# Orca0917/TransformerTTS

Measured on AMD Instinct MI355X. Metric: mel frames/sec teacher-forced step, LJSpeech-shape batch, 1/2/4/8 MI355X, higher is better.
Workload: dtype f32

## Files before the change

### include/ttts_hip.h

```cpp
#ifndef TTTS_HIP_H
#define TTTS_HIP_H

#include <stddef.h>
#include <stdint.h>

#ifdef __cplusplus
extern "C" {
#endif

#define TTTS_OK 0
#define TTTS_ERR_INVALID (-1)
#define TTTS_ERR_LAUNCH (-2)

#define TTTS_AMAX_SLOTS 1024

#define TTTS_ACT_NONE 0
#define TTTS_ACT_RELU 1
#define TTTS_ACT_TANH 2

typedef struct ttts_step_state {
    uint64_t seed;
    float lr;
    float p_tf;
    int64_t step;
// ... 225 lines not shown
                       size_t ws_bytes, int64_t* durations, uint8_t* valid, void* stream);
int ttts_heads_pad_w(const float* src, int64_t ld_src, float* dst, int64_t rows, int H, int head_dim, int width, void* stream);
int ttts_heads_unpad_w(const float* src, float* dst, int64_t ld_dst, int64_t rows, int H, int head_dim, int width, void* stream);
int ttts_attention_fwd_img(const void* q, const void* k, const void* v, const float* q_inv, const float* k_inv,
                           const float* v_inv, float* o, float* lse, float* attn, const int64_t* key_lens, int B, int H, int Tq,
                           int Tk, int ldq, int ldk, int ldv, int ldo, int causal, float q_scale, float drop_p, uint64_t seed,
                           const uint64_t* step_seed, const float* v_amax, float* o_amax_out, float* rowstat_out, int64_t q_inv_rows, int64_t k_inv_rows, int64_t stat_plane,
                           void* stream);
int ttts_attention_bwd_img(const void* q, const void* k, const void* v, const float* q_inv, const float* k_inv,
                           const float* v_inv, const float* o, const float* d_o, const float* rowstat, float* delta, float* dq,
                           float* dk, float* dv, const int64_t* key_lens, int B, int H, int Tq, int Tk, int ldq, int ldk, int ldv,
                           int ldo, int lddq, int lddk, int lddv, int causal, float q_scale, float drop_p, uint64_t seed,
                           const uint64_t* step_seed, const float* do_amax, float* dq_amax_out, float* dkv_amax_out,
                           float* dkv_partials , int q_splits ,
                           int64_t q_inv_rows, int64_t k_inv_rows, int64_t stat_plane, void* stream);

int ttts_embedding_fwd(const int64_t* ids, const float* table, float* out, int64_t n, int vocab, int d,
                       float* out_amax_out , void* stream);
int ttts_embedding_bwd(const int64_t* ids, const float* dout, float* dtable, int64_t n, int vocab, int d, int accumulate,
                       void* stream);
int ttts_posenc_fwd(const float* x, const float* pe, const float* alpha, float* y, int B, int T, int d, float drop_p,
                    uint64_t seed, const uint64_t* step_seed, float* y_amax_out , void* stream);
size_t ttts_posenc_bwd_workspace_bytes(void);
int ttts_posenc_bwd(const float* dy, const float* pe, float* dx, float* dalpha, float* ws, size_t ws_bytes, int B, int T,
                    int d, float drop_p, uint64_t seed, const uint64_t* step_seed, int accumulate, void* stream);
int ttts_relu_dropout_bwd(const float* dy, const float* out, float* dx, int64_t n, float drop_p, float* dx_amax_out,
                          void* stream);
int ttts_dropout_bwd(const float* dy, float* dx, int64_t n, float drop_p, uint64_t seed, const uint64_t* step_seed,
                     float* dx_amax_out, void* stream);
int ttts_zero(void* p, size_t nbytes, void* stream);
// ... 71 lines not shown
```

### transformertts_amd/_lib.py

```python
from __future__ import annotations

import ctypes
import os
from ctypes import c_char_p, c_float, c_int, c_int64, c_size_t, c_uint64, c_void_p

import torch

_HERE = os.path.dirname(os.path.abspath(__file__))
LIB_PATH = os.environ.get("TTTS_LIB", os.path.join(_HERE, "libttts_hip.so"))

P, I, L, F, U, Z = c_void_p, c_int, c_int64, c_float, c_uint64, c_size_t

SIGNATURES = {
    "ttts_last_error": (c_char_p, []),
    "ttts_abi_version": (I, []),
    "ttts_linear_fwd": (I, [P, P, P, P, P, L, I, I, I, F, U, P, I, I, P]),
    "ttts_linear_bwd_data": (I, [P, P, P, P, L, I, I, P, F, P]),
    "ttts_wgrad_workspace_bytes": (Z, [L, I, I, I]),
    "ttts_linear_bwd_weight": (I, [P, P, P, P, P, Z, L, I, I, I, I, I, P, P]),
    "ttts_split_bytes": (Z, [L, L]),
    "ttts_split_image_bytes": (Z, [L, L, I, I, I]),
    "ttts_gemm_tile_choice": (I, [L, I, I, I]),
    "ttts_weight_split": (I, [P, P, I, I, I, I, I, P]),
    "ttts_weight_split_units": (L, [L, L, I, I]),
# ... 37 lines not shown
    "ttts_bn_apply_fwd": (I, [P, P, P, P, P, P, L, I, I, F, U, P, P, P]),
    "ttts_bn_bwd": (I, [P, P, P, P, P, P, P, P, P, P, Z, L, I, I, F, U, P, I, P, I, P]),
    "ttts_layernorm_fwd": (I, [P, P, P, P, P, P, L, I, F, P, P, P, P]),
    "ttts_layernorm_bwd_workspace_bytes": (Z, [I]),
    "ttts_layernorm_bwd": (I, [P, P, P, P, P, P, P, P, P, Z, L, I, I, P, P, P, P]),
    "ttts_layernorm_bwd_drop": (I, [P, P, P, P, P, P, P, P, P, Z, L, I, I, P, F, U, P, P, P, P, P, P]),
    "ttts_attention_fwd": (I, [P, P, P, P, P, P, P, I, I, I, I, I, I, I, I, I, F, F, U, P, P]),
    "ttts_attention_fwd_x6": (I, [P, P, P, P, P, P, P, I, I, I, I, I, I, I, I, I, F, F, U, P, P]),
    "ttts_attention_fwd_h3": (I, [P, P, P, P, P, P, P, I, I, I, I, I, I, I, I, I, F, F, U, P, P, P, P, P, P, P]),
    "ttts_attention_bwd": (I, [P, P, P, P, P, P, P, P, P, P, P, I, I, I, I, I, I, I, I, I, I, I, I, F, F, U, P, P]),
    "ttts_attention_bwd_x6": (I, [P, P, P, P, P, P, P, P, P, P, P, I, I, I, I, I, I, I, I, I, I, I, I, F, F, U, P, P]),
    "ttts_attention_bwd_h3": (I, [P, P, P, P, P, P, P, P, P, P, P, I, I, I, I, I, I, I, I, I, I, I, I, F, F, U, P, P, P, P, P, P, P, P, P]),
    "ttts_attention_fwd_img": (I, [P, P, P, P, P, P, P, P, P, P, I, I, I, I, I, I, I, I, I, F, F, U, P, P, P, P, L, L, L, P]),
    "ttts_attention_bwd_img": (I, [P, P, P, P, P, P, P, P, P, P, P, P, P, P, I, I, I, I, I, I, I, I, I, I, I, I, F, F, U, P, P, P, P,
                                   P, I, L, L, L, P]),
    "ttts_attention_fwd_wide": (I, [P, P, P, P, P, P, P, I, I, I, I, I, I, I, I, I, F, F, U, P, P]),
    "ttts_attention_bwd_wide": (I, [P, P, P, P, P, P, P, P, P, P, P, I, I, I, I, I, I, I, I, I, I, I, I, F, F, U, P, P]),
    "ttts_attention_fwd_wide_masked": (I, [P, P, P, P, P, P, P, I, I, I, I, I, I, I, I, I, F, F, U, P, P, L, L, L, P, L, P]),
    "ttts_attention_bwd_wide_masked": (I, [P, P, P, P, P, P, P, P, P, P, P, I, I, I, I, I, I, I, I, I, I, I, I, F, F, U, P, P, L, L, L,
                                           P, L, P]),
    "ttts_attention_bwd_wide_dattn": (I, [P, P, P, P, P, P, P, P, P, P, P, I, I, I, I, I, I, I, I, I, I, I, I, F, F, U, P, P, L, L, L,
                                          P, L, P, P, L, L, L, P]),
    "ttts_guided_attention_fwd": (I, [P, P, P, U, F, I, I, I, I, P, I, I, I, P, P]),
    "ttts_guided_attention_bwd": (I, [P, P, P, U, F, I, I, I, I, I, I, P, P]),
    "ttts_alignment_rowstats": (I, [P, L, L, L, P, P, I, I, I, I, I, I, P, P, P, P]),
    "ttts_alignment_select": (I, [P, P, P, I, I, I, I, I, I, P, P, P]),
    "ttts_alignment_durations_argmax": (I, [P, P, P, P, I, I, I, I, I, P, P, P]),
    "ttts_alignment_mas_workspace_bytes": (Z, [I, I, I]),
    "ttts_alignment_mas": (I, [P, I, L, L, L, P, P, P, I, I, I, I, P, Z, P, P, P]),
    "ttts_heads_pad": (I, [P, L, P, L, I, I, P]),
# ... 76 lines not shown
```

### transformertts_amd/csrc/attention_common.h

```cpp
#pragma once
#include "ttts_common.h"

namespace ttts {

constexpr int HD = 64;
constexpr int KT_LD = HD + 1;
constexpr int WHD = 128;
constexpr int WLD = WHD + 1;
constexpr int QB = 128;
constexpr float NEG_INF = -__builtin_inff();
__device__ __forceinline__ float fast_exp2(float x) { return __builtin_amdgcn_exp2f(x); }
typedef unsigned int u32x4v __attribute__((ext_vector_type(4)));

struct RowSrc {
    __amdgpu_buffer_rsrc_t rsrc;
    int ld;
};
__device__ __forceinline__ RowSrc row_src(const float* base, long nrows, int ld) {
    RowSrc r;
    r.rsrc = __builtin_amdgcn_make_buffer_rsrc(const_cast<float*>(base), 0, (uint32_t)(nrows * ld * 4), 0x00020000);
    r.ld = ld;
    return r;
}
__device__ __forceinline__ float4 row_load4(const RowSrc& s, long row, int c4) {
// ... 209 lines not shown
    float m = 0.f;
#pragma unroll
    for (int r = 0; r < 16; ++r) m = fmaxf(m, fabsf(ds[r]));
    m = fmaxf(m, __shfl_xor(m, 32, 64));
    const uint32_t e = (__float_as_uint(m) >> 23) & 0xffu;
    const bool change = e >= 24u && e < 255u && (sds == 0.f || m * sds > 8192.f);
    if (__any(change)) {
        const float snew = change ? __uint_as_float((265u - e) << 23) : sds;
        const float f = (change && sds != 0.f) ? snew / sds : 1.f;
#pragma unroll
        for (int r = 0; r < 16; ++r) { acc[0][r] *= f; acc[1][r] *= f; }
        sds = snew;
    }
}

__device__ __forceinline__ void load_lane_frags_h3(const float* scratch, int l31, int half, float scale, f16x8v (&f)[4][2]) {
#pragma unroll
    for (int st = 0; st < 4; ++st) {
        float x[8];
#pragma unroll
        for (int e = 0; e < 8; ++e) x[e] = scratch[l31 * KT_LD + 16 * st + 8 * half + e];
        split_frag8_h3(x, scale, f[st][0], f[st][1]);
    }
}

static inline int attn_check(const char* name, int width, int B, int H, int Tq, int Tk, int ldq, int ldk, int ldv, int ldo,
                             int causal, float drop_p) {
    TTTS_REQUIRE(B > 0 && H > 0 && Tq > 0 && Tk > 0, "%s: sizes must be positive (B %d, H %d, Tq %d, Tk %d)", name, B, H, Tq, Tk);
    TTTS_REQUIRE((long)B * H < (1L << 31) && cdiv(Tq, QB) <= 65535 && cdiv(Tk, QB) <= 65535,
                 "%s: grid too large (B*H %ld, Tq %d, Tk %d)", name, (long)B * H, Tq, Tk);
// ... 59 lines not shown
```

### transformertts_amd/csrc/attention_img.hip

```cpp
#include "attention_common.h"

namespace ttts {

struct AttnImgArgs {
    const void* q; const void* k; const void* v;
    const float* q_inv; const float* k_inv; const float* v_inv;
    long q_rows, k_rows;
    long stat_plane;
    float* o; float* lse; float* attn;
    const float* dout; float* delta; float* dq; float* dk; float* dv;
    const int64_t* key_lens;
    int B, H, Tq, Tk;
    int ldq, ldk, ldv, ldo, lddq, lddk, lddv;
    float qscale;
    float drop_scale; uint32_t thr; uint64_t seed; const uint64_t* step_seed;
    const float* v_amax;
    const float* do_amax;
    float* amax_dq; float* amax_dkv;
    float* dkv_part; long part_stride;
    int ldp;
    float* o_amax;
    float* rowstat;
};

__device__ __forceinline__ uint32_t lds_addr_a(const void* p) {
    return (uint32_t)(uintptr_t)(__attribute__((address_space(3))) const void*)p;
}
typedef unsigned int u32x4a __attribute__((ext_vector_type(4)));
__device__ __forceinline__ void dma16a(u32x4a rsrc, uint32_t voff, uint32_t soff, uint32_t lds_dst) {
    uint32_t keep;
    asm volatile("s_mov_b32 %0, m0\n\ts_mov_b32 m0, %3\n\ts_nop 0\n\tbuffer_load_dwordx4 %1, %2, %4 offen lds\n\ts_mov_b32 m0, %0"
                 : "=&s"(keep) : "v"(voff), "s"(rsrc), "s"(lds_dst), "s"(soff) : "memory");
}
__device__ __forceinline__ void dma4a(u32x4a rsrc, uint32_t voff, uint32_t lds_dst) {
    uint32_t keep;
    asm volatile("s_mov_b32 %0, m0\n\ts_mov_b32 m0, %3\n\ts_nop 0\n\tbuffer_load_dword %1, %2, 0 offen lds\n\ts_mov_b32 m0, %0"
                 : "=&s"(keep) : "v"(voff), "s"(rsrc), "s"(lds_dst) : "memory");
}
__device__ __forceinline__ u32x4a make_rsrc(const void* base, uint32_t bytes) {
    const uint64_t a = reinterpret_cast<uint64_t>(base);
    return u32x4a{(uint32_t)a, (uint32_t)(a >> 32) & 0xffffu, bytes, 0x00020000u};
}

constexpr int IMG_PLANE = 64 * 128;
constexpr int IMG_TILE = 2 * IMG_PLANE;
__device__ __forceinline__ int isw(int r) { return ((r & 2) << 1) | ((r >> 2) & 3); }
typedef short s16x4v __attribute__((ext_vector_type(4)));
__device__ __forceinline__ s16x4v lds_tr4(const char* p) {
    return __builtin_amdgcn_ds_read_tr16_b64_v4i16(
        (__attribute__((address_space(3))) s16x4v*)(uintptr_t)lds_addr_a(p));
}
// ... 792 lines not shown
        const float fin = (sds > 0.f) ? a.qscale / sds : 0.f;
        float mx = 0.f;
#pragma unroll
        for (int r = 0; r < 16; ++r) {
            dq[0][r] *= fin; dq[1][r] *= fin;
            mx = fmaxf(mx, fmaxf(fabsf(dq[0][r]), fabsf(dq[1][r])));
        }
        if (a.amax_dq != nullptr) amax_publish(qg < a.Tq ? mx : 0.f, a.amax_dq, blockIdx.y * gridDim.x + blockIdx.x);
    }
    wave_store_rows4(dq, scratch4, a.dq + (long)b * a.Tq * a.lddq + h * HD, qw0, a.Tq, a.lddq, lane);
}

constexpr int DKI_QS = 32;
constexpr int DKI_PLANE = DKI_QS * 128;
constexpr int DKI_STAGE = 4 * DKI_PLANE + 5 * 256;
template <bool CAUSAL>
__global__ __launch_bounds__(256, 2) void attn_bwd_dkv_img_kernel(AttnImgArgs a) {
    const uint64_t seed_eff = site_seed(a.seed, a.step_seed);
    const uint32_t thr16 = a.thr << 16;
    __shared__ __attribute__((aligned(16))) char xs[(2 * DKI_STAGE > OUT_BYTES) ? 2 * DKI_STAGE : OUT_BYTES];
    __shared__ float red4[4];

    const int tid = threadIdx.x, lane = tid & 63;
    const int wave = __builtin_amdgcn_readfirstlane(tid >> 6);
    const int l31 = lane & 31, half = lane >> 5;
    const int kblk = blockIdx.y;
    const int h = blockIdx.x % a.H, b = blockIdx.x / a.H;
    const int k0 = kblk * QB, kw0 = k0 + wave * 32;
    const int kg = kw0 + l31;
    const uint32_t key_mult = attn_drop_mult((uint32_t)kg);
    float* scratch4 = reinterpret_cast<float*>(xs) + wave * 32 * OUT_LD;
// ... 14 lines not shown
#pragma unroll
            for (int p = 0; p < 2; ++p) {
                kf[s][p] = *reinterpret_cast<const f16x8v*>(kp + p * 128 + (2 * s + half) * 16);
                vf[s][p] = *reinterpret_cast<const f16x8v*>(vp + p * 128 + (2 * s + half) * 16);
            }
    }
    const float kinv = a.k_inv[(long)h * a.k_rows + (long)b * a.Tk + krow];
    const float vinv = a.v_inv[(long)h * a.k_rows + (long)b * a.Tk + krow];

    f32x16 dk[2], dv[2];
#pragma unroll
    for (int r = 0; r < 16; ++r) { dk[0][r] = 0.f; dk[1][r] = 0.f; dv[0][r] = 0.f; dv[1][r] = 0.f; }

    const float dp_unscale = inv_g * vinv * a.drop_scale;
    float sds = 0.f;
    const int nqs_all = (a.Tq + DKI_QS - 1) / DKI_QS;
    const int per_z = (nqs_all + (int)gridDim.z - 1) / (int)gridDim.z;
    const int nqs = min(nqs_all, ((int)blockIdx.z + 1) * per_z);
    int qs_begin = max(attn_qs_begin<CAUSAL, DKI_QS>(k0, klen, nqs), (int)blockIdx.z * per_z);
    if (qs_begin > nqs) qs_begin = nqs;

    const u32x4a rsQ = make_rsrc(reinterpret_cast<const char*>(a.q) + ((long)AIMG_SB(b) * a.Tq * a.ldq + AIMG_SH(h) * HD) * 4, (uint32_t)a.Tq * (uint32_t)a.ldq * 4u);
    const u32x4a rsG = make_rsrc(a.dout + (long)AIMG_SB(b) * a.Tq * a.ldo + AIMG_SH(h) * HD, (uint32_t)a.Tq * (uint32_t)a.ldo * 4u);
    const long plane = a.stat_plane;
    const u32x4a rsS0 = make_rsrc(a.rowstat + arow, (uint32_t)a.Tq * 4u), rsS1 = make_rsrc(a.rowstat + plane + arow, (uint32_t)a.Tq * 4u);
    const u32x4a rsS3 = make_rsrc(a.rowstat + 3 * plane + arow, (uint32_t)a.Tq * 4u), rsS4 = make_rsrc(a.rowstat + 4 * plane + arow, (uint32_t)a.Tq * 4u);
    const u32x4a rsD = make_rsrc(a.delta + arow, (uint32_t)a.Tq * 4u);
    const uint32_t lds0 = lds_addr_a(xs);
    const int ld_r = lane >> 3;
    const uint32_t ld_cq = (uint32_t)((lane & 7) ^ isw(8 * (wave & 1) + ld_r)) * 16u;
// ... 127 lines not shown
                const float4 f4 = *reinterpret_cast<const float4*>(stat + 256 + 2 * r + 4 * half);
                const float dl4[4] = {d4.x, d4.y, d4.z, d4.w}, cq4[4] = {f4.x, f4.y, f4.z, f4.w};
#pragma unroll
                for (int e = 0; e < 4; ++e) {
                    float g = dp[r + e] * dp_unscale;
                    float pk = pd[r + e];
                    {
                        const bool keep = attn_keep_word(hq[e], key_mult, thr16);
                        g = keep ? g : 0.f;
                        pk = keep ? pk : 0.f;
                    }
                    ds[r + e] = pd[r + e] * (g - dl4[e]) * cq4[e];
                    pd[r + e] = pk;
                }
            }
            attn_h3_track_scale(ds, sds, dk);
#pragma unroll
            for (int t2 = 0; t2 < 2; ++t2) {
                float x[8];
                f16x8v f[2];
#pragma unroll
                for (int e = 0; e < 8; ++e) x[e] = pd[8 * t2 + e];
                split_frag8_h3(x, H3A_P, f[0], f[1]);
#pragma unroll
                for (int i2 = 0; i2 < 2; ++i2) {
                    f16x8v af[2];
#pragma unroll
                    for (int pl = 0; pl < 2; ++pl) {
                        const char* gb = st_ + (2 + pl) * DKI_PLANE + t2 * 2048;
                        af[pl] = join_tr(lds_tr4(gb + t_off[i2][0]), lds_tr4(gb + t_off[i2][1]));
// ... 42 lines not shown

__global__ __launch_bounds__(256) void attn_dkv_reduce_kernel(const float* __restrict__ part, float* __restrict__ out, long n4, int zs,
                                                              long stride, float* __restrict__ amax, int cols4, long out_ld) {
    float mx = 0.f;
    for (long i = (long)blockIdx.x * blockDim.x + threadIdx.x; i < n4; i += (long)gridDim.x * blockDim.x) {
        float4 acc = reinterpret_cast<const float4*>(part)[i];
        for (int z = 1; z < zs; ++z) {
            const float4 v = reinterpret_cast<const float4*>(part + (long)z * stride)[i];
            acc.x += v.x; acc.y += v.y; acc.z += v.z; acc.w += v.w;
        }
        const long row = i / cols4;
        *reinterpret_cast<float4*>(out + row * out_ld + (i - row * cols4) * 4) = acc;
        mx = fmaxf(fmaxf(mx, fmaxf(fabsf(acc.x), fabsf(acc.y))), fmaxf(fabsf(acc.z), fabsf(acc.w)));
    }
    if (amax != nullptr) amax_publish(mx, amax, blockIdx.x * 4 + (threadIdx.x >> 6));
}

#ifndef TTTS_AIMG_KT
#define TTTS_AIMG_KT 32
#endif

static int check_img_spans(const char* name, int Tq, int Tk, int ldq, int ldk, int ldv) {
    TTTS_REQUIRE((uint64_t)Tq * ldq * 4 < (1ull << 32) && (uint64_t)Tk * ldk * 4 < (1ull << 32) && (uint64_t)Tk * ldv * 4 < (1ull << 32),
                 "%s: one utterance's operand exceeds 4 GiB", name);
    return TTTS_OK;
}
static int fill_img_planes(const char* name, AttnImgArgs& a, int B, int H, int Tq, int Tk, int64_t q_inv_rows, int64_t k_inv_rows,
                           int64_t stat_plane) {
    TTTS_REQUIRE((q_inv_rows == 0 || q_inv_rows >= (int64_t)B * Tq) && (k_inv_rows == 0 || k_inv_rows >= (int64_t)B * Tk) &&
                 (stat_plane == 0 || stat_plane >= (int64_t)B * H * Tq), "%s: plane strides smaller than the batch", name);
// ... 32 lines not shown
    a.o = o; a.lse = lse; a.attn = attn;
    a.v_amax = v_amax; a.o_amax = o_amax_out; a.rowstat = rowstat_out;
    dim3 grid(B * H, cdiv(Tq, QB), 1);
    if (causal)
        hipLaunchKernelGGL((attn_fwd_img_kernel<true, false, TTTS_AIMG_KT>), grid, dim3(256), 0, (hipStream_t)stream, a);
    else if (!attn)
        hipLaunchKernelGGL((attn_fwd_img_kernel<false, false, TTTS_AIMG_KT>), grid, dim3(256), 0, (hipStream_t)stream, a);
    else if (Tk <= 128)
        hipLaunchKernelGGL(attn_fwd_img_maps_kernel, grid, dim3(256), 0, (hipStream_t)stream, a);
    else
        hipLaunchKernelGGL((attn_fwd_img_kernel<false, true, 64>), grid, dim3(256), 0, (hipStream_t)stream, a);
    TTTS_LAUNCH_CHECK("attn_fwd_img_kernel");
    return TTTS_OK;
}

extern "C" int ttts_attention_bwd_img(const void* q, const void* k, const void* v, const float* q_inv, const float* k_inv,
                                      const float* v_inv, const float* o, const float* d_o, const float* rowstat, float* delta,
                                      float* dq, float* dk, float* dv, const int64_t* key_lens, int B, int H, int Tq, int Tk, int ldq,
                                      int ldk, int ldv, int ldo, int lddq, int lddk, int lddv, int causal, float q_scale,
                                      float drop_p, uint64_t seed, const uint64_t* step_seed, const float* do_amax,
                                      float* dq_amax_out, float* dkv_amax_out, float* dkv_partials, int q_splits,
                                      int64_t q_inv_rows, int64_t k_inv_rows, int64_t stat_plane, void* stream_) {
    hipStream_t stream = (hipStream_t)stream_;
    TTTS_REQUIRE(q && k && v && q_inv && k_inv && v_inv && o && d_o && rowstat && delta && dq && dk && dv && key_lens && do_amax,
                 "attention_bwd_img: null pointer");
    int rc = attn_check("attention_bwd_img", HD, B, H, Tq, Tk, ldq, ldk, ldv, ldo, causal, drop_p);
    if (!rc) rc = check_img_spans("attention_bwd_img", Tq, Tk, ldq, ldk, ldv);
    if (!rc) rc = attn_check_grad_strides("attention_bwd_img", HD, H, lddq, lddk, lddv);
    if (rc) return rc;
    TTTS_REQUIRE((((uintptr_t)q | (uintptr_t)k | (uintptr_t)v | (uintptr_t)o | (uintptr_t)d_o | (uintptr_t)do_amax) & 15) == 0,
                 "attention_bwd_img: q/k/v/o/d_o/do_amax must be 16-byte aligned");
    TTTS_REQUIRE((uint64_t)Tq * ldo * 4 < (1ull << 32), "attention_bwd_img: one utterance's d_o exceeds 4 GiB");
    AttnImgArgs a = {};
    attn_fill(a, key_lens, B, H, Tq, Tk, ldq, ldk, ldv, ldo, q_scale, drop_p, seed, step_seed);
    rc = fill_img_planes("attention_bwd_img", a, B, H, Tq, Tk, q_inv_rows, k_inv_rows, stat_plane);
    if (rc) return rc;
    a.q = q; a.k = k; a.v = v; a.q_inv = q_inv; a.k_inv = k_inv; a.v_inv = v_inv;
    a.o = const_cast<float*>(o); a.dout = d_o; a.delta = delta; a.dq = dq; a.dk = dk; a.dv = dv;
    a.lddq = lddq; a.lddk = lddk; a.lddv = lddv;
    a.do_amax = do_amax; a.amax_dq = dq_amax_out; a.amax_dkv = dkv_amax_out;
    a.rowstat = const_cast<float*>(rowstat);
    TTTS_REQUIRE(q_splits >= 1 && q_splits <= 16, "attention_bwd_img: q_splits out of 1..16");
    if (q_splits > 1) {
        TTTS_REQUIRE(dkv_partials && dv == dk + H * HD && lddk >= 2 * H * HD && lddv == lddk,
                     "attention_bwd_img: query splits need a workspace and a (dk | dv) gradient whose rows hold dk then dv");
        a.ldp = 2 * H * HD;
        a.dkv_part = dkv_partials; a.part_stride = (long)B * Tk * a.ldp;
    }
    rc = ATTN_LAUNCH_BWD(attn_bwd_dq_img_kernel, 0, attn_bwd_dkv_img_kernel, 0, causal, "attention_bwd_img", "attn_bwd_dq_img_kernel",
                         "attn_bwd_dkv_img_kernel", a, q_splits, stream);
    if (rc) return rc;
    if (q_splits > 1) {
        const long n4 = a.part_stride / 4;
        const long blocks = (n4 + 255) / 256;
        hipLaunchKernelGGL(attn_dkv_reduce_kernel, dim3((unsigned)(blocks < 2048 ? blocks : 2048)), dim3(256), 0, stream, dkv_partials, dk, n4,
                           q_splits, a.part_stride, dkv_amax_out, a.ldp / 4, (long)lddk);
        TTTS_LAUNCH_CHECK("attn_dkv_reduce_kernel");
    }
    return TTTS_OK;
}
```

### transformertts_amd/csrc/elementwise.hip

```cpp
#include <stdarg.h>

#include "ttts_common.h"

namespace ttts {

static thread_local char g_err[512] = "";
void set_error(const char* fmt, ...) {
    va_list ap;
    va_start(ap, fmt);
    vsnprintf(g_err, sizeof(g_err), fmt, ap);
    va_end(ap);
}

static inline int ew_grid(long n_items) {
    long g = (n_items + 255) / 256;
    if (g > 2048) g = 2048;
    if (g < 1) g = 1;
    return (int)g;
}

__global__ __launch_bounds__(256) void zero_kernel(uint32_t* __restrict__ p, long n) {
    const long head = (long)(((16 - (reinterpret_cast<uintptr_t>(p) & 15)) & 15) >> 2) < n ? (long)(((16 - (reinterpret_cast<uintptr_t>(p) & 15)) & 15) >> 2) : n;
    const long n4 = (n - head) / 4;
    uint4* q = reinterpret_cast<uint4*>(p + head);
// ... 311 lines not shown
    if (lane == 0) red[wave][1024] = accb;
    __syncthreads();
    for (int c = threadIdx.x; c < d; c += 256)
        ws[(long)blockIdx.x * (d + 1) + c] = (red[0][c] + red[1][c]) + (red[2][c] + red[3][c]);
    if (threadIdx.x == 0)
        ws[(long)blockIdx.x * (d + 1) + d] = (red[0][1024] + red[1][1024]) + (red[2][1024] + red[3][1024]);
}

}

using namespace ttts;

extern "C" {

const char* ttts_last_error(void) { return ttts::g_err; }
int ttts_abi_version(void) { return 21; }

int ttts_zero(void* p, size_t nbytes, void* stream) { return ::ttts::launch_zero(p, nbytes, (hipStream_t)stream); }

int ttts_heads_pad(const float* src, int64_t ld_src, float* dst, int64_t rows, int H, int head_dim, void* stream) {
    TTTS_REQUIRE(src && dst && rows > 0 && H > 0 && head_dim > 0 && head_dim <= 64 && ld_src >= (int64_t)H * head_dim,
                 "heads_pad: bad arguments (head_dim %d must be in 1..64)", head_dim);
    hipLaunchKernelGGL(heads_pad_kernel<64>, dim3(ew_grid(rows * H * 64)), dim3(256), 0, (hipStream_t)stream, src, (long)ld_src, dst,
                       (long)rows, H, head_dim, 0, 0L);
    TTTS_LAUNCH_CHECK("heads_pad_kernel");
    return TTTS_OK;
}

int ttts_heads_unpad(const float* src, float* dst, int64_t ld_dst, int64_t rows, int H, int head_dim, void* stream) {
    TTTS_REQUIRE(src && dst && rows > 0 && H > 0 && head_dim > 0 && head_dim <= 64 && ld_dst >= (int64_t)H * head_dim,
                 "heads_unpad: bad arguments (head_dim %d must be in 1..64)", head_dim);
// ... 144 lines not shown
```

### transformertts_amd/ops.py

```python
from __future__ import annotations

import os
import weakref
from ctypes import c_void_p
from typing import Optional

import torch

from . import _lib

ACT_NONE, ACT_RELU, ACT_TANH = 0, 1, 2
AMAX_SLOTS = 1024


def _p(t: Optional[torch.Tensor]):
    return None if t is None else c_void_p(t.data_ptr())


_raw_stream = getattr(torch._C, "_cuda_getCurrentRawStream", None)


def _stream():
    if _raw_stream is not None:
        return c_void_p(_raw_stream(torch.cuda.current_device()))
# ... 1580 lines not shown


def _img_operand(cells: torch.Tensor, himg: "HeadImage", col: int):
    return _off(cells, col), cells.stride(1), himg.inv_of(col), himg.row_inv.shape[1]


def _attn_img_fwd(q, k, v, o, stat, attn, lens, B, H, Tq, Tk, causal, drop_p, seed, v_am, o_am) -> None:
    lib = _lib.load()
    (qp, ldq, qi, q_rows), (kp, ldk, ki, k_rows), (vp, ldv, vi, _) = q, k, v
    _lib.check(lib.ttts_attention_fwd_img(qp, kp, vp, qi, ki, vi, _p(o), _p(stat[0]), _p(attn), _p(lens), B, H, Tq, Tk, ldq, ldk,
                                          ldv, o.shape[-1], 1 if causal else 0, 0.125, float(drop_p), seed, _ss(), _p(v_am),
                                          _p(o_am), _p(stat[1:]), q_rows, k_rows, stat.stride(0), _stream()),
               "ttts_attention_fwd_img")


def _attn_img_bwd(q, k, v, o, do, stat, delta, dq, dk, dv, lens, B, H, Tq, Tk, causal, drop_p, seed, ss, dq_am, dkv_am,
                  partials=None, q_splits: int = 1) -> None:
    lib = _lib.load()
    (qp, ldq, qi, q_rows), (kp, ldk, ki, k_rows), (vp, ldv, vi, _) = q, k, v
    _lib.check(lib.ttts_attention_bwd_img(qp, kp, vp, qi, ki, vi, _p(o), _p(do), _p(stat[1:]), _p(delta), dq[0], dk[0], dv[0],
                                          _p(lens), B, H, Tq, Tk, ldq, ldk, ldv, o.shape[-1], dq[1], dk[1], dv[1],
                                          1 if causal else 0, 0.125, drop_p, seed, ss, _p(_amax(do)), _p(dq_am), _p(dkv_am),
                                          _p(partials), q_splits, q_rows, k_rows, stat.stride(0), _stream()),
               "ttts_attention_bwd_img")


def _head_width(d: int, n_head: int) -> int:
    if n_head <= 0 or d % n_head != 0:
        raise ValueError(f"attention: d_model {d} is not divisible by {n_head} heads")
    return d // n_head


def masked_attention(q, k, v, lens, n_head: int, causal: bool, drop_p: float, dead=None, add_mask=None):
    B, Tq, d = q.shape
# ... 614 lines not shown
```

Measured before the change: 4.123 million.

## Hand dS tiles from dK/dV kernel to a lightweight dQ kernel in attention backward

Adds a backward path where the dK/dV kernel writes its dS tiles to a global workspace, and a new dQ kernel reads them back and multiplies by K instead of recomputing QK^T, softmax and dP. A separate delta kernel computes the row dot products and the d_o amax first. The path is on by default whenever the workspace fits under a 2 GiB cap. This trades recomputation for extra global memory traffic and workspace (B*H*Tq*Tk floats). It also raises an s_nop in the LDS DMA helper.

```diff
diff --git a/include/ttts_hip.h b/include/ttts_hip.h
--- a/include/ttts_hip.h
+++ b/include/ttts_hip.h
@@ -263,6 +263,16 @@
                            const uint64_t* step_seed, const float* do_amax, float* dq_amax_out, float* dkv_amax_out,
                            float* dkv_partials , int q_splits ,
                            int64_t q_inv_rows, int64_t k_inv_rows, int64_t stat_plane, void* stream);
+size_t ttts_attention_ds_workspace_bytes(int B, int H, int Tq, int Tk, int causal);
+int ttts_attention_ds_handoff(int causal);
+int ttts_attention_bwd_img_ds(const void* q, const void* k, const void* v, const float* q_inv, const float* k_inv,
+                              const float* v_inv, const float* o, const float* d_o, const float* rowstat, float* delta, float* dq,
+                              float* dk, float* dv, const int64_t* key_lens, int B, int H, int Tq, int Tk, int ldq, int ldk, int ldv,
+                              int ldo, int lddq, int lddk, int lddv, int causal, float q_scale, float drop_p, uint64_t seed,
+                              const uint64_t* step_seed, float* do_amax, float* dq_amax_out, float* dkv_amax_out,
+                              float* dkv_partials , int q_splits ,
+                              int64_t q_inv_rows, int64_t k_inv_rows, int64_t stat_plane, float* ds_workspace,
+                              size_t ds_workspace_bytes, void* stream);
 
 int ttts_embedding_fwd(const int64_t* ids, const float* table, float* out, int64_t n, int vocab, int d,
                        float* out_amax_out , void* stream);
diff --git a/transformertts_amd/_lib.py b/transformertts_amd/_lib.py
--- a/transformertts_amd/_lib.py
+++ b/transformertts_amd/_lib.py
@@ -75,6 +75,10 @@
     "ttts_attention_fwd_img": (I, [P, P, P, P, P, P, P, P, P, P, I, I, I, I, I, I, I, I, I, F, F, U, P, P, P, P, L, L, L, P]),
     "ttts_attention_bwd_img": (I, [P, P, P, P, P, P, P, P, P, P, P, P, P, P, I, I, I, I, I, I, I, I, I, I, I, I, F, F, U, P, P, P, P,
                                    P, I, L, L, L, P]),
+    "ttts_attention_ds_workspace_bytes": (Z, [I, I, I, I, I]),
+    "ttts_attention_ds_handoff": (I, [I]),
+    "ttts_attention_bwd_img_ds": (I, [P, P, P, P, P, P, P, P, P, P, P, P, P, P, I, I, I, I, I, I, I, I, I, I, I, I, F, F, U, P, P, P,
+                                      P, P, I, L, L, L, P, Z, P]),
     "ttts_attention_fwd_wide": (I, [P, P, P, P, P, P, P, I, I, I, I, I, I, I, I, I, F, F, U, P, P]),
     "ttts_attention_bwd_wide": (I, [P, P, P, P, P, P, P, P, P, P, P, I, I, I, I, I, I, I, I, I, I, I, I, F, F, U, P, P]),
     "ttts_attention_fwd_wide_masked": (I, [P, P, P, P, P, P, P, I, I, I, I, I, I, I, I, I, F, F, U, P, P, L, L, L, P, L, P]),
diff --git a/transformertts_amd/csrc/attention_common.h b/transformertts_amd/csrc/attention_common.h
--- a/transformertts_amd/csrc/attention_common.h
+++ b/transformertts_amd/csrc/attention_common.h
@@ -247,6 +247,14 @@
     }
 }
 
+constexpr int DS_TILE_FLOATS = 32 * 32;
+constexpr int DS_TILE_BYTES = DS_TILE_FLOATS * 4;
+template <bool CAUSAL>
+__device__ __forceinline__ bool ds_tile_live(int kb, int qb, int klen, int Tq) {
+    return 32 * kb < klen && 32 * qb < Tq && (!CAUSAL || kb <= qb);
+}
+__host__ __device__ __forceinline__ long ds_tiles_per_head(int Tq, int Tk) { return (long)((Tk + 31) / 32) * ((Tq + 31) / 32); }
+
 __device__ __forceinline__ void load_lane_frags_h3(const float* scratch, int l31, int half, float scale, f16x8v (&f)[4][2]) {
 #pragma unroll
     for (int st = 0; st < 4; ++st) {
diff --git a/transformertts_amd/csrc/attention_img.hip b/transformertts_amd/csrc/attention_img.hip
--- a/transformertts_amd/csrc/attention_img.hip
+++ b/transformertts_amd/csrc/attention_img.hip
@@ -21,6 +21,7 @@
     int ldp;
     float* o_amax;
     float* rowstat;
+    float* ds_ws; long ds_head;
 };
 
 __device__ __forceinline__ uint32_t lds_addr_a(const void* p) {
@@ -34,7 +35,7 @@
 }
 __device__ __forceinline__ void dma4a(u32x4a rsrc, uint32_t voff, uint32_t lds_dst) {
     uint32_t keep;
-    asm volatile("s_mov_b32 %0, m0\n\ts_mov_b32 m0, %3\n\ts_nop 0\n\tbuffer_load_dword %1, %2, 0 offen lds\n\ts_mov_b32 m0, %0"
+    asm volatile("s_mov_b32 %0, m0\n\ts_mov_b32 m0, %3\n\ts_nop 2\n\tbuffer_load_dword %1, %2, 0 offen lds\n\ts_mov_b32 m0, %0"
                  : "=&s"(keep) : "v"(voff), "s"(rsrc), "s"(lds_dst) : "memory");
 }
 __device__ __forceinline__ u32x4a make_rsrc(const void* base, uint32_t bytes) {
@@ -857,7 +858,7 @@
 constexpr int DKI_QS = 32;
 constexpr int DKI_PLANE = DKI_QS * 128;
 constexpr int DKI_STAGE = 4 * DKI_PLANE + 5 * 256;
-template <bool CAUSAL>
+template <bool CAUSAL, bool WRITE_DS = false>
 __global__ __launch_bounds__(256, 2) void attn_bwd_dkv_img_kernel(AttnImgArgs a) {
     const uint64_t seed_eff = site_seed(a.seed, a.step_seed);
     const uint32_t thr16 = a.thr << 16;
@@ -902,6 +903,9 @@
 
     const float dp_unscale = inv_g * vinv * a.drop_scale;
     float sds = 0.f;
+    [[maybe_unused]] float* ds_lane = nullptr;
+    if constexpr (WRITE_DS)
+        ds_lane = a.ds_ws + (long)blockIdx.x * a.ds_head + (long)(kw0 >> 5) * ((a.Tq + 31) >> 5) * DS_TILE_FLOATS + 16 * lane;
     const int nqs_all = (a.Tq + DKI_QS - 1) / DKI_QS;
     const int per_z = (nqs_all + (int)gridDim.z - 1) / (int)gridDim.z;
     const int nqs = min(nqs_all, ((int)blockIdx.z + 1) * per_z);
@@ -1059,6 +1063,11 @@
                     pd[r + e] = pk;
                 }
             }
+            if constexpr (WRITE_DS) {
+                float4* dst = reinterpret_cast<float4*>(ds_lane + (long)qs * DS_TILE_FLOATS);
+#pragma unroll
+                for (int g4 = 0; g4 < 4; ++g4) dst[g4] = make_float4(ds[4 * g4], ds[4 * g4 + 1], ds[4 * g4 + 2], ds[4 * g4 + 3]);
+            }
             attn_h3_track_scale(ds, sds, dk);
 #pragma unroll
             for (int t2 = 0; t2 < 2; ++t2) {
@@ -1131,6 +1140,166 @@
         mx = fmaxf(fmaxf(mx, fmaxf(fabsf(acc.x), fabsf(acc.y))), fmaxf(fabsf(acc.z), fabsf(acc.w)));
     }
     if (amax != nullptr) amax_publish(mx, amax, blockIdx.x * 4 + (threadIdx.x >> 6));
+}
+
+
+__global__ __launch_bounds__(256) void attn_bwd_delta_img_kernel(AttnImgArgs a, float* __restrict__ do_amax_out) {
+    __shared__ float xs[SMEM_FLOATS];
+    const int tid = threadIdx.x, lane = tid & 63;
+    const int wave = __builtin_amdgcn_readfirstlane(tid >> 6);
+    const int l31 = lane & 31, half = lane >> 5;
+    const int h = blockIdx.x % a.H, b = blockIdx.x / a.H;
+    const int qw0 = blockIdx.y * QB + wave * 32;
+    const int qg = qw0 + l31;
+    float* scratch = xs + wave * 32 * KT_LD;
+    const float* ob_ = a.o + (long)b * a.Tq * a.ldo + h * HD;
+    const float* gb_ = a.dout + (long)b * a.Tq * a.ldo + h * HD;
+    const long arow = ((long)(b * a.H + h) * a.Tq);
+
+    wave_stage_tile(ob_, qw0, a.Tq, a.ldo, lane, scratch, 1.f);
+    wave_lds_sync();
+    float orow[32];
+#pragma unroll
+    for (int j = 0; j < 32; ++j) orow[j] = scratch[l31 * KT_LD + 2 * j + half];
+    wave_lds_sync();
+    wave_stage_tile(gb_, qw0, a.Tq, a.ldo, lane, scratch, 1.f);
+    wave_lds_sync();
+    float delta = 0.f, gmax = 0.f;
+#pragma unroll
+    for (int j = 0; j < 32; ++j) {
+        const float g = scratch[l31 * KT_LD + 2 * j + half];
+        delta += g * orow[j];
+        gmax = fmaxf(gmax, fabsf(g));
+    }
+    delta += __shfl_xor(delta, 32, 64);
+    if (half == 0 && qg < a.Tq) {
+        const long plane = a.stat_plane;
+        const bool saturated = a.rowstat[2 * plane + arow + qg] != 0.f;
+        a.delta[arow + qg] = saturated ? -0.f : delta;
+        if (saturated) a.rowstat[4 * plane + arow + qg] = 0.f;
+    }
+    amax_publish(gmax, do_amax_out, (blockIdx.y * gridDim.x + blockIdx.x) * 4 + wave);
+}
+
+constexpr int DQS_KT = 32;
+constexpr int DQS_KPL = DQS_KT * 128;
+constexpr int DQS_DS = 2 * DQS_KPL + 256;
+constexpr int DQS_STAGE = DQS_DS + 4 * DS_TILE_BYTES;
+static_assert(2 * DQS_STAGE >= OUT_BYTES, "the epilogue's scratch aliases the stages");
+template <bool CAUSAL>
+__global__ __launch_bounds__(256, 3) void attn_bwd_dq_ds_kernel(AttnImgArgs a) {
+    __shared__ __attribute__((aligned(16))) char xs[2 * DQS_STAGE];
+
+    const int tid = threadIdx.x, lane = tid & 63;
+    const int wave = __builtin_amdgcn_readfirstlane(tid >> 6);
+    const int l31 = lane & 31, half = lane >> 5;
+    const int qblk = CAUSAL ? (gridDim.y - 1 - blockIdx.y) : blockIdx.y;
+    const int h = blockIdx.x % a.H, b = blockIdx.x / a.H;
+    const int q0 = qblk * QB, qw0 = q0 + wave * 32;
+    const int qg = qw0 + l31, qb = qw0 >> 5;
+    float* scratch4 = reinterpret_cast<float*>(xs) + wave * 32 * OUT_LD;
+
+    const int klen = attn_klen(a.key_lens, b, a.Tk);
+    const int nst = key_range<CAUSAL, false, DQS_KT>(klen, a.Tk, q0, qw0).nst;
+    const int nqb = (a.Tq + 31) >> 5;
+
+    const int qrow = qg < a.Tq ? qg : a.Tq - 1;
+    const float qinv = a.q_inv[(long)h * a.q_rows + (long)b * a.Tq + qrow];
+    float sds = 0.f;
+    f32x16 dq[2];
+#pragma unroll
+    for (int r = 0; r < 16; ++r) { dq[0][r] = 0.f; dq[1][r] = 0.f; }
+
+    const u32x4a rsK = make_rsrc(reinterpret_cast<const char*>(a.k) + ((long)b * a.Tk * a.ldk + h * HD) * 4, (uint32_t)a.Tk * (uint32_t)a.ldk * 4u);
+    const u32x4a rsKi = make_rsrc(a.k_inv + (long)h * a.k_rows + (long)b * a.Tk, (uint32_t)a.Tk * 4u);
+    const u32x4a rsD = make_rsrc(a.ds_ws + (long)blockIdx.x * a.ds_head, (uint32_t)(a.ds_head * 4));
+    const uint32_t lds0 = lds_addr_a(xs);
+    const int ld_r = lane >> 3;
+    const uint32_t ld_ck = (uint32_t)((lane & 7) ^ isw(8 * (wave & 1) + ld_r)) * 16u;
+    const uint32_t ld_cd = (uint32_t)(2048 * ((lane >> 2) & 1) + 64 * (4 * ((lane >> 3) & 1) + (lane >> 4)) + 16 * (lane & 3));
+    auto issue = [&](int t, int stage) {
+        const uint32_t dst = lds0 + (uint32_t)stage * DQS_STAGE;
+        int row = t * DQS_KT + 8 * wave + ld_r;
+        row = row < a.Tk ? row : a.Tk - 1;
+        const uint32_t ko = (uint32_t)row * (uint32_t)(a.ldk * 4) + ld_ck;
+#pragma unroll
+        for (int p = 0; p < 2; ++p)
+            dma16a(rsK, ko, (uint32_t)p * 128u, __builtin_amdgcn_readfirstlane(dst + (uint32_t)p * DQS_KPL + (uint32_t)(8 * wave) * 128u));
+        if (wave == 0) {
+            int key = t * DQS_KT + lane;
+            key = key < a.Tk ? key : a.Tk - 1;
+            dma4a(rsKi, (uint32_t)key * 4u, __builtin_amdgcn_readfirstlane(dst + 2 * DQS_KPL));
+        }
+        if (ds_tile_live<CAUSAL>(t, qb, klen, a.Tq)) {
+            const uint32_t so = (uint32_t)(t * nqb + qb) * (uint32_t)DS_TILE_BYTES + ld_cd;
+#pragma unroll
+            for (int i = 0; i < 4; ++i)
+                dma16a(rsD, so, 512u * i, __builtin_amdgcn_readfirstlane(dst + DQS_DS + (uint32_t)wave * DS_TILE_BYTES + 1024u * i));
+        }
+    };
+    auto landed = [&]() { asm volatile("s_waitcnt vmcnt(0)\n\ts_barrier" ::: "memory"); };
+
+    const uint32_t d_off = (uint32_t)(DQS_DS + wave * DS_TILE_BYTES + 128 * half + 64 * ((l31 >> 2) & 1) + 16 * (l31 >> 3) + 4 * (l31 & 3));
+    const int q4 = (lane & 15) >> 2, pc = lane & 3, g16 = (lane >> 4) & 1;
+    uint32_t kt_off[2][2];
+#pragma unroll
+    for (int i2 = 0; i2 < 2; ++i2)
+#pragma unroll
+        for (int sc = 0; sc < 2; ++sc) {
+            const int r = 8 * sc + 4 * half + q4;
+            const int ch = 4 * i2 + 2 * g16 + (pc >> 1);
+            kt_off[i2][sc] = (uint32_t)(r * 128 + ((ch ^ isw(r)) << 4) + (pc & 1) * 8);
+        }
+
+    if (nst > 0) issue(0, 0);
+    landed();
+    for (int t = 0; t < nst; ++t) {
+        if (t + 1 < nst) issue(t + 1, (t + 1) & 1);
+        const char* st_ = xs + (t & 1) * DQS_STAGE;
+        if (ds_tile_live<CAUSAL>(t, qb, klen, a.Tq)) {
+            const float* ki = reinterpret_cast<const float*>(st_ + 2 * DQS_KPL) + 4 * half;
+            float ds[16];
+#pragma unroll
+            for (int g4 = 0; g4 < 4; ++g4) {
+                const float4 f = *reinterpret_cast<const float4*>(ki + 8 * g4);
+                const float kf4[4] = {f.x, f.y, f.z, f.w};
+#pragma unroll
+                for (int e = 0; e < 4; ++e)
+                    ds[4 * g4 + e] = *reinterpret_cast<const float*>(st_ + d_off + 256 * (4 * g4 + e)) * kf4[e];
+            }
+            attn_h3_track_scale(ds, sds, dq);
+#pragma unroll
+            for (int t2 = 0; t2 < 2; ++t2) {
+                float x[8];
+#pragma unroll
+                for (int e = 0; e < 8; ++e) x[e] = ds[8 * t2 + e];
+                f16x8v dsf[2];
+                split_frag8_h3(x, sds, dsf[0], dsf[1]);
+#pragma unroll
+                for (int i2 = 0; i2 < 2; ++i2) {
+                    f16x8v ktf[2];
+#pragma unroll
+                    for (int pl = 0; pl < 2; ++pl) {
+                        const char* kb = st_ + pl * DQS_KPL + t2 * 2048;
+                        ktf[pl] = join_tr(lds_tr4(kb + kt_off[i2][0]), lds_tr4(kb + kt_off[i2][1]));
+                    }
+                    mfma_h3(dq[i2], ktf, dsf);
+                }
+            }
+        }
+        landed();
+    }
+    {
+        const float fin = (sds > 0.f) ? 1.f / (qinv * sds) : 0.f;
+        float mx = 0.f;
+#pragma unroll
+        for (int r = 0; r < 16; ++r) {
+            dq[0][r] *= fin; dq[1][r] *= fin;
+            mx = fmaxf(mx, fmaxf(fabsf(dq[0][r]), fabsf(dq[1][r])));
+        }
+        if (a.amax_dq != nullptr) amax_publish(qg < a.Tq ? mx : 0.f, a.amax_dq, blockIdx.y * gridDim.x + blockIdx.x);
+    }
+    wave_store_rows4(dq, scratch4, a.dq + (long)b * a.Tq * a.lddq + h * HD, qw0, a.Tq, a.lddq, lane);
 }
 
 #ifndef TTTS_AIMG_KT
@@ -1193,48 +1362,104 @@
     return TTTS_OK;
 }
 
+static int attention_bwd_img_body(const char* name, const void* q, const void* k, const void* v, const float* q_inv, const float* k_inv,
+                                  const float* v_inv, const float* o, const float* d_o, const float* rowstat, float* delta, float* dq,
+                                  float* dk, float* dv, const int64_t* key_lens, int B, int H, int Tq, int Tk, int ldq, int ldk,
+                                  int ldv, int ldo, int lddq, int lddk, int lddv, int causal, float q_scale, float drop_p,
+                                  uint64_t seed, const uint64_t* step_seed, const float* do_amax, float* dq_amax_out,
+                                  float* dkv_amax_out, float* dkv_partials, int q_splits, int64_t q_inv_rows, int64_t k_inv_rows,
+                                  int64_t stat_plane, float* ds_ws, hipStream_t stream) {
+    TTTS_REQUIRE(q && k && v && q_inv && k_inv && v_inv && o && d_o && rowstat && delta && dq && dk && dv && key_lens && do_amax,
+                 "%s: null pointer", name);
+    int rc = attn_check(name, HD, B, H, Tq, Tk, ldq, ldk, ldv, ldo, causal, drop_p);
+    if (!rc) rc = check_img_spans(name, Tq, Tk, ldq, ldk, ldv);
+    if (!rc) rc = attn_check_grad_strides(name, HD, H, lddq, lddk, lddv);
+    if (rc) return rc;
+    TTTS_REQUIRE((((uintptr_t)q | (uintptr_t)k | (uintptr_t)v | (uintptr_t)o | (uintptr_t)d_o | (uintptr_t)do_amax) & 15) == 0,
+                 "%s: q/k/v/o/d_o/do_amax must be 16-byte aligned", name);
+    TTTS_REQUIRE((uint64_t)Tq * ldo * 4 < (1ull << 32), "%s: one utterance's d_o exceeds 4 GiB", name);
+    AttnImgArgs a = {};
+    attn_fill(a, key_lens, B, H, Tq, Tk, ldq, ldk, ldv, ldo, q_scale, drop_p, seed, step_seed);
+    rc = fill_img_planes(name, a, B, H, Tq, Tk, q_inv_rows, k_inv_rows, stat_plane);
+    if (rc) return rc;
+    a.q = q; a.k = k; a.v = v; a.q_inv = q_inv; a.k_inv = k_inv; a.v_inv = v_inv;
+    a.o = const_cast<float*>(o); a.dout = d_o; a.delta = delta; a.dq = dq; a.dk = dk; a.dv = dv;
+    a.lddq = lddq; a.lddk = lddk; a.lddv = lddv;
+    a.do_amax = do_amax; a.amax_dq = dq_amax_out; a.amax_dkv = dkv_amax_out;
+    a.rowstat = const_cast<float*>(rowstat);
+    TTTS_REQUIRE(q_splits >= 1 && q_splits <= 16, "%s: q_splits out of 1..16", name);
+    if (q_splits > 1) {
+        TTTS_REQUIRE(dkv_partials && dv == dk + H * HD && lddk >= 2 * H * HD && lddv == lddk,
+                     "%s: query splits need a workspace and a (dk | dv) gradient whose rows hold dk then dv", name);
+        a.ldp = 2 * H * HD;
+        a.dkv_part = dkv_partials; a.part_stride = (long)B * Tk * a.ldp;
+    }
+    const dim3 grid_q(B * H, cdiv(Tq, QB), 1), grid_k(B * H, cdiv(Tk, QB), q_splits);
+    if (ds_ws == nullptr) {
+        rc = ATTN_LAUNCH_BWD(attn_bwd_dq_img_kernel, 0, attn_bwd_dkv_img_kernel, 0, causal, name, "attn_bwd_dq_img_kernel",
+                             "attn_bwd_dkv_img_kernel", a, q_splits, stream);
+        if (rc) return rc;
+    } else {
+        a.ds_ws = ds_ws; a.ds_head = ds_tiles_per_head(Tq, Tk) * DS_TILE_FLOATS;
+        TTTS_REQUIRE((uint64_t)a.ds_head * 4 < (1ull << 32), "%s: one head's dS tiles exceed 4 GiB", name);
+        hipLaunchKernelGGL(attn_bwd_delta_img_kernel, grid_q, dim3(256), 0, stream, a, const_cast<float*>(do_amax));
+        TTTS_LAUNCH_CHECK("attn_bwd_delta_img_kernel");
+        if (causal) hipLaunchKernelGGL((attn_bwd_dkv_img_kernel<true, true>), grid_k, dim3(256), 0, stream, a);
+        else hipLaunchKernelGGL((attn_bwd_dkv_img_kernel<false, true>), grid_k, dim3(256), 0, stream, a);
+        TTTS_LAUNCH_CHECK("attn_bwd_dkv_img_kernel");
+    }
+    if (q_splits > 1) {
+        const long n4 = a.part_stride / 4;
+        const long blocks = (n4 + 255) / 256;
+        hipLaunchKernelGGL(attn_dkv_reduce_kernel, dim3((unsigned)(blocks < 2048 ? blocks : 2048)), dim3(256), 0, stream, dkv_partials, dk, n4,
+                           q_splits, a.part_stride, dkv_amax_out, a.ldp / 4, (long)lddk);
+        TTTS_LAUNCH_CHECK("attn_dkv_reduce_kernel");
+    }
+    if (ds_ws != nullptr) {
+        if (causal) hipLaunchKernelGGL(attn_bwd_dq_ds_kernel<true>, grid_q, dim3(256), 0, stream, a);
+        else hipLaunchKernelGGL(attn_bwd_dq_ds_kernel<false>, grid_q, dim3(256), 0, stream, a);
+        TTTS_LAUNCH_CHECK("attn_bwd_dq_ds_kernel");
+    }
+    return TTTS_OK;
+}
+
 extern "C" int ttts_attention_bwd_img(const void* q, const void* k, const void* v, const float* q_inv, const float* k_inv,
                                       const float* v_inv, const float* o, const float* d_o, const float* rowstat, float* delta,
                                       float* dq, float* dk, float* dv, const int64_t* key_lens, int B, int H, int Tq, int Tk, int ldq,
                                       int ldk, int ldv, int ldo, int lddq, int lddk, int lddv, int causal, float q_scale,
                                       float drop_p, uint64_t seed, const uint64_t* step_seed, const float* do_amax,
                                       float* dq_amax_out, float* dkv_amax_out, float* dkv_partials, int q_splits,
-                                      int64_t q_inv_rows, int64_t k_inv_rows, int64_t stat_plane, void* stream_) {
-    hipStream_t stream = (hipStream_t)stream_;
-    TTTS_REQUIRE(q && k && v && q_inv && k_inv && v_inv && o && d_o && rowstat && delta && dq && dk && dv && key_lens && do_amax,
-                 "attention_bwd_img: null pointer");
-    int rc = attn_check("attention_bwd_img", HD, B, H, Tq, Tk, ldq, ldk, ldv, ldo, causal, drop_p);
-    if (!rc) rc = check_img_spans("attention_bwd_img", Tq, Tk, ldq, ldk, ldv);
-    if (!rc) rc = attn_check_grad_strides("attention_bwd_img", HD, H, lddq, lddk, lddv);
-    if (rc) return rc;
-    TTTS_REQUIRE((((uintptr_t)q | (uintptr_t)k | (uintptr_t)v | (uintptr_t)o | (uintptr_t)d_o | (uintptr_t)do_amax) & 15) == 0,
-                 "attention_bwd_img: q/k/v/o/d_o/do_amax must be 16-byte aligned");
-    TTTS_REQUIRE((uint64_t)Tq * ldo * 4 < (1ull << 32), "attention_bwd_img: one utterance's d_o exceeds 4 GiB");
-    AttnImgArgs a = {};
-    attn_fill(a, key_lens, B, H, Tq, Tk, ldq, ldk, ldv, ldo, q_scale, drop_p, seed, step_seed);
-    rc = fill_img_planes("attention_bwd_img", a, B, H, Tq, Tk, q_inv_rows, k_inv_rows, stat_plane);
-    if (rc) return rc;
-    a.q = q; a.k = k; a.v = v; a.q_inv = q_inv; a.k_inv = k_inv; a.v_inv = v_inv;
-    a.o = const_cast<float*>(o); a.dout = d_o; a.delta = delta; a.dq = dq; a.dk = dk; a.dv = dv;
-    a.lddq = lddq; a.lddk = lddk; a.lddv = lddv;
-    a.do_amax = do_amax; a.amax_dq = dq_amax_out; a.amax_dkv = dkv_amax_out;
-    a.rowstat = const_cast<float*>(rowstat);
-    TTTS_REQUIRE(q_splits >= 1 && q_splits <= 16, "attention_bwd_img: q_splits out of 1..16");
-    if (q_splits > 1) {
-        TTTS_REQUIRE(dkv_partials && dv == dk + H * HD && lddk >= 2 * H * HD && lddv == lddk,
-                     "attention_bwd_img: query splits need a workspace and a (dk | dv) gradient whose rows hold dk then dv");
-        a.ldp = 2 * H * HD;
-        a.dkv_part = dkv_partials; a.part_stride = (long)B * Tk * a.ldp;
-    }
-    rc = ATTN_LAUNCH_BWD(attn_bwd_dq_img_kernel, 0, attn_bwd_dkv_img_kernel, 0, causal, "attention_bwd_img", "attn_bwd_dq_img_kernel",
-                         "attn_bwd_dkv_img_kernel", a, q_splits, stream);
-    if (rc) return rc;
-    if (q_splits > 1) {
-        const long n4 = a.part_stride / 4;
-        const long blocks = (n4 + 255) / 256;
-        hipLaunchKernelGGL(attn_dkv_reduce_kernel, dim3((unsigned)(blocks < 2048 ? blocks : 2048)), dim3(256), 0, stream, dkv_partials, dk, n4,
-                           q_splits, a.part_stride, dkv_amax_out, a.ldp / 4, (long)lddk);
-        TTTS_LAUNCH_CHECK("attn_dkv_reduce_kernel");
-    }
-    return TTTS_OK;
-}
+                                      int64_t q_inv_rows, int64_t k_inv_rows, int64_t stat_plane, void* stream) {
+    return attention_bwd_img_body("attention_bwd_img", q, k, v, q_inv, k_inv, v_inv, o, d_o, rowstat, delta, dq, dk, dv, key_lens, B, H, Tq,
+                                  Tk, ldq, ldk, ldv, ldo, lddq, lddk, lddv, causal, q_scale, drop_p, seed, step_seed, do_amax, dq_amax_out,
+                                  dkv_amax_out, dkv_partials, q_splits, q_inv_rows, k_inv_rows, stat_plane, nullptr, (hipStream_t)stream);
+}
+
+extern "C" size_t ttts_attention_ds_workspace_bytes(int B, int H, int Tq, int Tk, int causal) {
+    (void)causal;
+    if (B <= 0 || H <= 0 || Tq <= 0 || Tk <= 0) return 0;
+    return (size_t)B * H * (size_t)ds_tiles_per_head(Tq, Tk) * DS_TILE_BYTES;
+}
+
+#ifndef TTTS_DS_HANDOFF_SITES
+#define TTTS_DS_HANDOFF_SITES 3
+#endif
+extern "C" int ttts_attention_ds_handoff(int causal) { return (TTTS_DS_HANDOFF_SITES >> (causal ? 0 : 1)) & 1; }
+
+extern "C" int ttts_attention_bwd_img_ds(const void* q, const void* k, const void* v, const float* q_inv, const float* k_inv,
+                                         const float* v_inv, const float* o, const float* d_o, const float* rowstat, float* delta,
+                                         float* dq, float* dk, float* dv, const int64_t* key_lens, int B, int H, int Tq, int Tk,
+                                         int ldq, int ldk, int ldv, int ldo, int lddq, int lddk, int lddv, int causal, float q_scale,
+                                         float drop_p, uint64_t seed, const uint64_t* step_seed, float* do_amax, float* dq_amax_out,
+                                         float* dkv_amax_out, float* dkv_partials, int q_splits, int64_t q_inv_rows,
+                                         int64_t k_inv_rows, int64_t stat_plane, float* ds_workspace, size_t ds_workspace_bytes,
+                                         void* stream) {
+    TTTS_REQUIRE(ds_workspace && ((uintptr_t)ds_workspace & 15) == 0, "attention_bwd_img_ds: the dS workspace must be a 16-byte aligned pointer");
+    TTTS_REQUIRE(ds_workspace_bytes >= ttts_attention_ds_workspace_bytes(B, H, Tq, Tk, causal),
+                 "attention_bwd_img_ds: the dS workspace has %zu bytes, %zu are needed", ds_workspace_bytes,
+                 ttts_attention_ds_workspace_bytes(B, H, Tq, Tk, causal));
+    return attention_bwd_img_body("attention_bwd_img_ds", q, k, v, q_inv, k_inv, v_inv, o, d_o, rowstat, delta, dq, dk, dv, key_lens, B, H,
+                                  Tq, Tk, ldq, ldk, ldv, ldo, lddq, lddk, lddv, causal, q_scale, drop_p, seed, step_seed, do_amax,
+                                  dq_amax_out, dkv_amax_out, dkv_partials, q_splits, q_inv_rows, k_inv_rows, stat_plane, ds_workspace,
+                                  (hipStream_t)stream);
+}
diff --git a/transformertts_amd/csrc/elementwise.hip b/transformertts_amd/csrc/elementwise.hip
--- a/transformertts_amd/csrc/elementwise.hip
+++ b/transformertts_amd/csrc/elementwise.hip
@@ -349,7 +349,7 @@
 extern "C" {
 
 const char* ttts_last_error(void) { return ttts::g_err; }
-int ttts_abi_version(void) { return 21; }
+int ttts_abi_version(void) { return 22; }
 
 int ttts_zero(void* p, size_t nbytes, void* stream) { return ::ttts::launch_zero(p, nbytes, (hipStream_t)stream); }
 
diff --git a/transformertts_amd/ops.py b/transformertts_amd/ops.py
--- a/transformertts_amd/ops.py
+++ b/transformertts_amd/ops.py
@@ -1618,10 +1618,27 @@
                "ttts_attention_fwd_img")
 
 
+ATTN_DS_HANDOFF = True
+ATTN_DS_CAP = 2 << 30
+
+
 def _attn_img_bwd(q, k, v, o, do, stat, delta, dq, dk, dv, lens, B, H, Tq, Tk, causal, drop_p, seed, ss, dq_am, dkv_am,
                   partials=None, q_splits: int = 1) -> None:
     lib = _lib.load()
     (qp, ldq, qi, q_rows), (kp, ldk, ki, k_rows), (vp, ldv, vi, _) = q, k, v
+    if ATTN_DS_HANDOFF and lib.ttts_attention_ds_handoff(1 if causal else 0):
+        nbytes = lib.ttts_attention_ds_workspace_bytes(B, H, Tq, Tk, 1 if causal else 0)
+        if nbytes <= ATTN_DS_CAP:
+            do_am = getattr(do, "_ttts_amax", None)
+            if do_am is None:
+                do_am = _amax_slots(do.device, True)
+            _lib.check(lib.ttts_attention_bwd_img_ds(qp, kp, vp, qi, ki, vi, _p(o), _p(do), _p(stat[1:]), _p(delta), dq[0], dk[0],
+                                                     dv[0], _p(lens), B, H, Tq, Tk, ldq, ldk, ldv, o.shape[-1], dq[1], dk[1], dv[1],
+                                                     1 if causal else 0, 0.125, drop_p, seed, ss, _p(do_am), _p(dq_am), _p(dkv_am),
+                                                     _p(partials), q_splits, q_rows, k_rows, stat.stride(0),
+                                                     _p(_ws(nbytes, do.device)), nbytes, _stream()),
+                       "ttts_attention_bwd_img_ds")
+            return
     _lib.check(lib.ttts_attention_bwd_img(qp, kp, vp, qi, ki, vi, _p(o), _p(do), _p(stat[1:]), _p(delta), dq[0], dk[0], dv[0],
                                           _p(lens), B, H, Tq, Tk, ldq, ldk, ldv, o.shape[-1], dq[1], dk[1], dv[1],
                                           1 if causal else 0, 0.125, drop_p, seed, ss, _p(_amax(do)), _p(dq_am), _p(dkv_am),
```

After: 4.122 million. No clear change (-0.0%).
